# zhb94430/RayTracer-Utah

Hardware: AMD Instinct MI355X
Metric: Mrays/sec at 1920x1080 (the reference's primary + secondary + shadow rays of the frames rendered / wall time; batched throughput: config.frames_in_flight frames with their own cameras per launch sequence — one frame alone: config.single_frame) (higher is better)
Workload: dtype f32

## Files before the change

### include/rtu_render.h

```cpp
#ifndef RTU_RENDER_H_INCLUDED
#define RTU_RENDER_H_INCLUDED

#include "rtu_scene.h"

#ifdef __cplusplus
extern "C" {
#endif

#define RTU_OK               0
#define RTU_ERR_ARG         (-1)
#define RTU_ERR_HIP         (-2)
#define RTU_ERR_UNSUPPORTED (-3)
#define RTU_ERR_STOCHASTIC  (-4)
#define RTU_ERR_NO_SCENE    (-5)
#define RTU_ERR_NO_DEVICE   (-6)
#define RTU_ERR_CAPACITY    (-7)
#define RTU_ERR_CANCELLED   (-8)
#define RTU_ERR_SCENE_SHAPE (-9)
#define RTU_ERR_STALE       (-10)

#define RTU_BAND_ROWS 8

typedef struct RtuContext RtuContext;

// ... 142 lines not shown
int  rtu_light_list_info(const RtuContext* ctx, uint32_t index, uint32_t* out5);

typedef struct RtuLightListDump {
    int32_t  usable, node, light;
    uint32_t G, point, n_entries;
    float    X[3], Y[3], Z[3], L[3], u0, v0, su, sv;
    uint32_t* cell_off;
    uint32_t* entry_face;
    float*    entry_zmin;
} RtuLightListDump;
int  rtu_debug_light_list(const RtuSceneDesc* scene, uint32_t light_slot, uint32_t cover_slot, RtuLightListDump* out);
void rtu_debug_light_list_free(RtuLightListDump* dump);
int  rtu_debug_context_light_list(RtuContext* ctx, uint32_t index, RtuLightListDump* out);
int  rtu_debug_update_timing(RtuContext* ctx, int on, float* ms_out5);
int  rtu_debug_mesh_update_timing(RtuContext* ctx, int on, float* ms_out4);

#define RTU_MESH_BVH4          0
#define RTU_MESH_BVH8          1
#define RTU_MESH_FAST_TRI      2
#define RTU_MESH_REF_TRI       3
#define RTU_MESH_REF_BVH       4
#define RTU_MESH_REF_ELEMENTS  5
#define RTU_MESH_V             6
#define RTU_MESH_VN            7
#define RTU_MESH_HEADER        8
#define RTU_MESH_FAST_ELEMENTS 9
typedef struct RtuMeshHeaderDump {
    float    bmin[3], bmax[3], scale;
    uint32_t n_bvh_nodes, any_empty_box;
} RtuMeshHeaderDump;
int  rtu_debug_context_mesh(RtuContext* ctx, uint32_t mesh, int which, void* out, size_t capacity_bytes, size_t* bytes_out);
int  rtu_debug_host_mesh(const RtuMesh* uploaded, const RtuMesh* now, int which, void* out, size_t capacity_bytes, size_t* bytes_out);

int  rtu_frame_counts(RtuContext* ctx, uint32_t* frames_out, uint32_t* deferred_out);

int  rtu_get_stats(RtuContext* ctx, RtuStats* stats);

#define RTU_KERNEL_SLOTS 40
typedef struct RtuTouched {
    uint64_t rays;
    uint64_t node_tests, mesh_box_tests, inner4, inner8, inner_ref, tri_tests, winners, xform_levels;
    uint64_t record_bytes;
    uint64_t bound_tests;
    uint64_t inline_shadow_rays;
} RtuTouched;
int         rtu_get_touched(RtuContext* ctx, RtuTouched* per_slot, int n_slots);
int         rtu_get_touched_launches(RtuContext* ctx, uint32_t* per_slot, int n_slots);
unsigned long long rtu_touched_bytes(const RtuTouched* t, int textured);
const char* rtu_kernel_slot_name(int slot);

int  rtu_probe_kernel(RtuContext* ctx, int slot);
int  rtu_probe_read(RtuContext* ctx, float* total_ms_out, int* launches_out);

int  rtu_time_render(RtuContext* ctx, const RtuFrameDesc* frame, void* d_rgbz, void* hip_stream,
                     int iters, float* avg_ms_out);

int  rtu_selftest_division(RtuContext* ctx, unsigned long long n_pairs, unsigned long long seed,
                           unsigned long long* mismatches_out);

int  rtu_selftest_primitives(RtuContext* ctx, unsigned long long n_rays, unsigned long long seed,
                             unsigned long long* mismatches_out);

#define RTU_TEXOP_ATAN2F     0
#define RTU_TEXOP_ASINF      1
#define RTU_TEXOP_SPHERE_UV  2
#define RTU_TEXOP_ENV_UVW    3
// ... 25 lines not shown
```

### raytracer-utah_amd/__init__.py

```python
import ctypes
import os

_PKG = os.path.dirname(os.path.abspath(__file__))
_LIB = os.path.join(_PKG, "lib")

RTU_BIGFLOAT = 1.0e30
RTU_BAND_ROWS = 8

RTU_OK = 0
RTU_ERR_ARG = -1
RTU_ERR_HIP = -2
RTU_ERR_UNSUPPORTED = -3
RTU_ERR_STOCHASTIC = -4
RTU_ERR_NO_SCENE = -5
RTU_ERR_NO_DEVICE = -6
RTU_ERR_CAPACITY = -7
RTU_ERR_CANCELLED = -8
RTU_ERR_SCENE_SHAPE = -9
RTU_ERR_STALE = -10


class RtuError(RuntimeError):
    def __init__(self, code, msg=""):
        self.code = code
# ... 77 lines not shown


def _load(name):
    path = os.path.join(_LIB, name)
    if not os.path.exists(path):
        raise ImportError("%s is missing: build the HIP extension first (__graft_entry__.build() or "
                          "`make -C raytracer-utah_amd`); there is no CPU fallback" % path)
    return ctypes.CDLL(path, mode=ctypes.RTLD_GLOBAL)


hip = _load("librtu_hip.so")
host = _load("librtu_host.so")

_P = ctypes.c_void_p
_I = ctypes.c_int


def _sig(lib, name, restype, *argtypes):
    fn = getattr(lib, name)
    fn.restype = restype
    fn.argtypes = list(argtypes)
    return fn


HIP_SYMBOLS = ["rtu_device_count", "rtu_error_string", "rtu_create_context", "rtu_destroy_context", "rtu_last_error",
               "rtu_upload_scene", "rtu_validate_scene", "rtu_frame_setup", "rtu_shard_rows", "rtu_shard_max_rows", "rtu_shard_global_row",
               "rtu_render_frame_device", "rtu_render_frames_device", "rtu_pack_image_device", "rtu_minmax_z_device", "rtu_pack_output_device", "rtu_render_frame", "rtu_frame_status", "rtu_render_timeline", "rtu_frame_counts", "rtu_timeline_exits", "rtu_mesh_info", "rtu_light_list_info", "rtu_debug_light_list", "rtu_update_scene", "rtu_multi_update_scene", "rtu_scene_shape_diff", "rtu_debug_context_light_list", "rtu_debug_update_timing", "rtu_debug_light_list_free", "rtu_debug_walk_stack_limit", "rtu_debug_node_bounds", "rtu_debug_flags", "rtu_set_sequences_in_flight", "rtu_debug_tail_from", "rtu_get_stats", "rtu_get_touched", "rtu_get_touched_launches", "rtu_touched_bytes", "rtu_kernel_slot_name", "rtu_probe_kernel", "rtu_probe_read", "rtu_time_render", "rtu_selftest_division", "rtu_selftest_primitives", "rtu_context_stream", "rtu_context_device", "rtu_context_sync", "rtu_host_alloc_pinned", "rtu_host_free_pinned", "rtu_copy_to_host_async", "rtu_device_alloc",
               "rtu_device_free", "rtu_copy_to_host", "rtu_device_info", "rtu_set_cancel_flag", "rtu_create_context_multi", "rtu_destroy_context_multi",
               "rtu_multi_size", "rtu_multi_context", "rtu_multi_last_error", "rtu_multi_upload_scene", "rtu_multi_render_frame", "rtu_multi_gather_kind",
               "rtu_adaptive_defaults", "rtu_render_frame_adaptive", "rtu_render_frame_adaptive_device", "rtu_debug_sample_images", "rtu_debug_texcoords",
               "rtu_debug_device_allocations", "rtu_progressive_begin", "rtu_progressive_advance", "rtu_progressive_status",
               "rtu_progressive_snapshot_device", "rtu_progressive_snapshot", "rtu_progressive_free", "rtu_debug_device_bytes",
               "rtu_update_meshes", "rtu_multi_update_meshes", "rtu_debug_context_mesh", "rtu_debug_host_mesh", "rtu_debug_mesh_update_timing",
               "rtu_trace_rays_device", "rtu_occluded_rays_device", "rtu_trace_rays", "rtu_occluded_rays", "rtu_camera_rays"]
_sig(hip, "rtu_device_count", _I)
_sig(hip, "rtu_error_string", ctypes.c_char_p, _I)
_sig(hip, "rtu_create_context", _P, _I, ctypes.POINTER(_I))
_sig(hip, "rtu_destroy_context", None, _P)
_sig(hip, "rtu_last_error", ctypes.c_char_p, _P)
_sig(hip, "rtu_upload_scene", _I, _P, _P)
_sig(hip, "rtu_validate_scene", _I, _P, ctypes.c_char_p, ctypes.c_size_t)
_sig(hip, "rtu_frame_setup", _I, ctypes.POINTER(RtuCamera), _I, _I, ctypes.POINTER(RtuFrameDesc))
_sig(hip, "rtu_shard_rows", _I, ctypes.POINTER(RtuFrameDesc))
_sig(hip, "rtu_shard_max_rows", _I, _I, _I)
_sig(hip, "rtu_shard_global_row", _I, ctypes.POINTER(RtuFrameDesc), _I)
_sig(hip, "rtu_render_frame_device", _I, _P, ctypes.POINTER(RtuFrameDesc), _P, _P)
_sig(hip, "rtu_render_frames_device", _I, _P, ctypes.POINTER(RtuFrameDesc), _I, _P, _P)
_sig(hip, "rtu_pack_image_device", _I, _P, _P, ctypes.c_size_t, _P, _P, _P)
_sig(hip, "rtu_minmax_z_device", _I, _P, _P, ctypes.c_size_t, _I, _P, _P)
_sig(hip, "rtu_pack_output_device", _I, _P, _P, ctypes.c_size_t, _I, _P, _P, _P)
_sig(hip, "rtu_render_frame", _I, _P, ctypes.POINTER(RtuFrameDesc), _P, ctypes.POINTER(RtuStats))
_sig(hip, "rtu_frame_status", _I, _P)
_sig(hip, "rtu_get_touched", _I, _P, ctypes.POINTER(RtuTouched), _I)
_sig(hip, "rtu_touched_bytes", ctypes.c_uint64, ctypes.POINTER(RtuTouched), _I)
_sig(hip, "rtu_get_touched_launches", _I, _P, ctypes.POINTER(ctypes.c_uint32), _I)
_sig(hip, "rtu_kernel_slot_name", ctypes.c_char_p, _I)
_sig(hip, "rtu_probe_kernel", _I, _P, _I)
_sig(hip, "rtu_probe_read", _I, _P, ctypes.POINTER(ctypes.c_float), ctypes.POINTER(_I))
_sig(hip, "rtu_debug_walk_stack_limit", _I, _P, ctypes.c_uint32)
_sig(hip, "rtu_debug_node_bounds", _I, _P, _I)
_sig(hip, "rtu_debug_flags", _I, _P, ctypes.c_uint32)
_sig(hip, "rtu_set_sequences_in_flight", _I, _P, _I)
_sig(hip, "rtu_debug_tail_from", _I, _P, _I)
_sig(hip, "rtu_timeline_exits", _I, _P, _I, _I, ctypes.POINTER(ctypes.c_double))
_sig(hip, "rtu_mesh_info", _I, _P, ctypes.c_uint32, ctypes.POINTER(ctypes.c_uint32))
_sig(hip, "rtu_light_list_info", _I, _P, ctypes.c_uint32, ctypes.POINTER(ctypes.c_uint32))
_sig(hip, "rtu_frame_counts", _I, _P, ctypes.POINTER(ctypes.c_uint32), ctypes.POINTER(ctypes.c_uint32))
_sig(hip, "rtu_render_timeline", _I, _P, ctypes.POINTER(RtuFrameDesc), _P, _I, ctypes.POINTER(_I), ctypes.POINTER(ctypes.c_double),
     ctypes.POINTER(ctypes.c_double))
_sig(hip, "rtu_get_stats", _I, _P, ctypes.POINTER(RtuStats))
_sig(hip, "rtu_time_render", _I, _P, ctypes.POINTER(RtuFrameDesc), _P, _P, _I, ctypes.POINTER(ctypes.c_float))
_sig(hip, "rtu_selftest_primitives", _I, _P, ctypes.c_ulonglong, ctypes.c_ulonglong, ctypes.POINTER(ctypes.c_ulonglong))
_sig(hip, "rtu_selftest_division", _I, _P, ctypes.c_ulonglong, ctypes.c_ulonglong, ctypes.POINTER(ctypes.c_ulonglong))
_sig(hip, "rtu_device_alloc", _P, _P, ctypes.c_size_t)
_sig(hip, "rtu_device_free", None, _P, _P)
_sig(hip, "rtu_copy_to_host", _I, _P, _P, _P, ctypes.c_size_t)


class RtuAdaptiveDesc(ctypes.Structure):
    _fields_ = [("min_samples", ctypes.c_int32), ("increment", ctypes.c_int32), ("target_variance", ctypes.c_float), ("max_batch", ctypes.c_int32)]


RTU_MAX_BATCH = 16
_sig(hip, "rtu_adaptive_defaults", _I, ctypes.POINTER(RtuAdaptiveDesc))
_sig(hip, "rtu_render_frame_adaptive", _I, _P, ctypes.POINTER(RtuFrameDesc), ctypes.POINTER(RtuAdaptiveDesc), _P, _P, ctypes.POINTER(RtuStats))
_sig(hip, "rtu_render_frame_adaptive_device", _I, _P, ctypes.POINTER(RtuFrameDesc), ctypes.POINTER(RtuAdaptiveDesc), _P, _P, _P)
_sig(hip, "rtu_debug_sample_images", _I, _P, ctypes.POINTER(RtuFrameDesc), _I, _I, _P)
_sig(hip, "rtu_debug_texcoords", _I, _P, _I, _I, _P, ctypes.c_ulonglong, _P)
_sig(hip, "rtu_debug_device_allocations", ctypes.c_ulonglong)
_sig(hip, "rtu_debug_device_bytes", ctypes.c_ulonglong)
_sig(hip, "rtu_progressive_begin", _P, _P, ctypes.POINTER(RtuFrameDesc), ctypes.POINTER(RtuAdaptiveDesc), ctypes.POINTER(_I))
_sig(hip, "rtu_progressive_advance", _I, _P, _I, _P)
_sig(hip, "rtu_progressive_status", _I, _P, ctypes.POINTER(ctypes.c_int32), ctypes.POINTER(ctypes.c_uint32))
_sig(hip, "rtu_progressive_snapshot_device", _I, _P, _P, _P, _P)
_sig(hip, "rtu_progressive_snapshot", _I, _P, _P, _P)
_sig(hip, "rtu_progressive_free", None, _P)
TEXOP_ATAN2F, TEXOP_ASINF, TEXOP_SPHERE_UV, TEXOP_ENV_UVW, TEXOP_TILE_CLAMP, TEXOP_TEXTURE, TEXOP_MAP = range(7)
TEXOP_IN = (2, 1, 3, 3, 3, 3, 3)
TEXOP_OUT = (1, 1, 3, 3, 3, 3, 3)

# ... 618 lines not shown
        if rc < 0:
            self._check(rc)
        order = {name: i for i, name in enumerate(self.TIMELINE_SLOTS)}
        rows = [(self.TIMELINE_SLOTS[slot[i]], t0[i], t1[i]) for i in range(rc)]
        return sorted(rows, key=lambda r: (r[0].startswith("k_combine"), -order[r[0]] if r[0].startswith("k_combine") else order[r[0]]))

    def timeline_exits(self, kernel):
        import numpy as np
        buf = (ctypes.c_double * 8192)()
        rc = hip.rtu_timeline_exits(self._h, self.TIMELINE_SLOTS.index(kernel), 8192, buf)
        if rc < 0:
            self._check(rc)
        return np.array(buf[:rc])

    def mesh_info(self, mesh=0):
        o = (ctypes.c_uint32 * 5)()
        self._check(hip.rtu_mesh_info(self._h, mesh, o))
        return dict(zip(("faces", "sah_depth", "stack4", "nodes4", "nodes8"), list(o)))

    def light_lists(self):
        out, i = [], 0
        while True:
            o = (ctypes.c_uint32 * 5)()
            if hip.rtu_light_list_info(self._h, i, o) != 0:
                return out
            out.append(dict(zip(("light", "cover", "G", "entries", "longest"), list(o))))
            i += 1

    def frame_counts(self):
        fr, de = (ctypes.c_uint32 * 6)(), (ctypes.c_uint32 * 7)()
        self._check(hip.rtu_frame_counts(self._h, fr, de))
        return list(fr), list(de)

    def time_render(self, frame, d_ptr, stream, iters):
        ms = ctypes.c_float(0)
        self._check(hip.rtu_time_render(self._h, ctypes.byref(frame), d_ptr, stream, iters, ctypes.byref(ms)))
        return ms.value

    def touched(self, textured=False):
        arr = (RtuTouched * KERNEL_SLOTS)()
        n = hip.rtu_get_touched(self._h, arr, KERNEL_SLOTS)
        if n < 0:
            self._check(n)
        nl = (ctypes.c_uint32 * KERNEL_SLOTS)()
        hip.rtu_get_touched_launches(self._h, nl, KERNEL_SLOTS)
        out = {}
        for k in range(n):
            d = arr[k].as_dict()
            if any(d.values()):
                d["bytes"] = int(hip.rtu_touched_bytes(ctypes.byref(arr[k]), 1 if textured else 0))
                d["launches"] = int(nl[k])
                out[hip.rtu_kernel_slot_name(k).decode()] = d
        return out

    def probe_kernel(self, slot_name):
        slot = -1
        if slot_name is not None:
            names = [hip.rtu_kernel_slot_name(k).decode() for k in range(KERNEL_SLOTS)]
            slot = names.index(slot_name)
        self._check(hip.rtu_probe_kernel(self._h, slot))

    def probe_read(self):
        ms, n = ctypes.c_float(0), _I(0)
        self._check(hip.rtu_probe_read(self._h, ctypes.byref(ms), ctypes.byref(n)))
        return ms.value, n.value

# ... 110 lines not shown
```

### raytracer-utah_amd/csrc/render_impl.h

```cpp
#ifndef RTU_RENDER_IMPL_H_INCLUDED
#define RTU_RENDER_IMPL_H_INCLUDED
#include "rtu_intersect.h"

namespace {

#define TEXD ((TEX & 1) != 0)
#define SMPD ((TEX & 2) != 0)
#define BATD ((TEX & 4) != 0)
#define GID ((TEX & 8) != 0)
#define CNTD ((TEX & 16) != 0)
#ifndef RTU_OCC_PRIMARY
#define RTU_OCC_PRIMARY __attribute__((amdgpu_waves_per_eu(4, 4)))
#endif
#ifndef RTU_OCC_PRIMARY_S
#define RTU_OCC_PRIMARY_S __attribute__((amdgpu_waves_per_eu(5, 5)))
#endif
#ifndef RTU_OCC_TRACE
#define RTU_OCC_TRACE __attribute__((amdgpu_waves_per_eu(5, 5)))
#endif
#ifndef RTU_OCC_WALK
#define RTU_OCC_WALK __attribute__((amdgpu_waves_per_eu(3, 3)))
#endif
#ifndef RTU_OCC_CONSUME
#define RTU_OCC_CONSUME
// ... 378 lines not shown
            if (GID) {
                a.gi_h[pix] = make_float4(h.p.x, h.p.y, h.p.z, h.z);
                a.gi_h[pix + a.gi_total] = make_float4(h.N.x, h.N.y, h.N.z, __uint_as_float((want ? 1u : 0u) | (h.front ? 2u : 0u) | ((uint32_t)(mid + 1) << 2)));
                a.gi_h[pix + 2u * (size_t)a.gi_total] = make_float4(ray.dir.x, ray.dir.y, ray.dir.z, __uint_as_float(smp.key));
                if (TEXD) a.gi_h[pix + 3u * (size_t)a.gi_total] = make_float4(h.uvw.x, h.uvw.y, h.uvw.z, 0.0f);
                RTU_BYTES(TEXD ? 64u : 48u);
                want = false;
            }
        }
    }
    if (GID) return;
    uint32_t info = 0;
    if (want) info = make_info<TEX>(a, mid, a.frame.max_bounce, h.front, ray.dir, h.p, h.N, h.uvw, smp);
    if (!STATS && INLINE_SHADE && !(a.dbg & 2048u) && __any(want && !(info & (RTU_FI_MAIN | RTU_FI_C)))) {
        const bool tryI = want && !(info & (RTU_FI_MAIN | RTU_FI_C));
        uint32_t lit = ~0u;
        bool ok = false;
        if (tryI) ok = shadows_inline<TEX>(a, info, h.p, lit, cnt);
        if (tryI && ok) {
            f3 direct = mk3(0, 0, 0);
            if (info & RTU_FI_SH) {
                const f3 cam_pos = BATD ? ld3(a.cam[sidx].pos) : ld3(a.frame.cam_pos);
                direct = direct_light<false, TEX>(a, info, h.p, h.N, h.uvw, cam_pos, direct, [&](uint32_t j) { return ((lit >> j) & 1u) ? 1.0f : 0.0f; });
            }
            a.out[pix] = make_float4(direct.x, direct.y, direct.z, h.z);
            RTU_BYTES(16u);
            want = false;
        }
    }
    if (!(a.dbg & 8u)) append_root<TEX>(a, want, shard, info, h.p, h.N, pix, ray.dir, h.z, h.uvw, cnt, !DEFER && !STATS);
    if (CNTD && !DEFER && !COOP && (a.dbg & 131072u) && valid) a.out[pix].x = (float)walk_units;
}

template <int STACK, bool STATS, int TEX>
__device__ __forceinline__ void primary_stage1(const KernelArgs& a, uint32_t n_tiles) {
    const Stamp stamp(a, RTU_TL_PRIMARY);
    __shared__ uint32_t s_stack_all[STATS ? 4 * STACK * 64 : 4];
    uint32_t* stk = s_stack_all + (STATS ? (threadIdx.x >> 6) * (STACK * 64) + (threadIdx.x & 63u) : 0);
    const uint32_t lane = threadIdx.x & 63u;
    Counters cnt = {};
    const uint32_t wave = (uint32_t)__builtin_amdgcn_readfirstlane((int)(threadIdx.x >> 6));
    for (uint32_t btile = blockIdx.x * 4u + wave; btile < n_tiles; btile += gridDim.x * 4u) {
        uint32_t sidx = (SMPD || BATD) ? btile / a.tiles_per_image : 0u;
        uint32_t tile = btile - sidx * a.tiles_per_image;
        bool lane_on = true;
        if constexpr (SMPD) {
            if (a.act_list != nullptr) {
                sidx = btile / a.act_n;
                const RTU_CONST uint32_t* ent = as_const(reinterpret_cast<const uint32_t*>(a.act_list)) + 4u * (size_t)(btile - sidx * a.act_n);
                tile = ent[0];
                lane_on = (((unsigned long long)ent[3] << 32 | ent[2]) >> lane) & 1ull;
            }
        }
        const uint32_t band_local = tile / a.tiles_x;
        const uint32_t tx = tile - band_local * a.tiles_x;
        const int x = (int)(tx * 8 + (lane & 7));
        const int ly = (int)(band_local * RTU_BAND_ROWS + (lane >> 3));
        const int y = (int)((band_local * a.frame.shard_count + a.frame.shard_rank) * RTU_BAND_ROWS + (lane >> 3));
        const bool valid = x < a.frame.width && y < a.frame.height && lane_on;
        const uint32_t pix = ((SMPD || BATD) ? sidx * a.batch_pixels : 0u) + (uint32_t)ly * (uint32_t)a.frame.width + (uint32_t)x;
        if (!STATS && !SMPD && !GID && a.occ != nullptr) {
            const uint32_t w = as_const(a.occ)[(size_t)sidx * a.occ_words + (tile >> 5)];
            if (!((w >> (tile & 31u)) & 1u)) {
                if (valid) {
                    const f3 bg = background_sample<TEXD>(a.scene, x, y);
                    a.out[pix] = make_float4(bg.x, bg.y, bg.z, RTU_BIGFLOAT);
                    RTU_BYTES(16u);
                    if (CNTD) cnt.t_rays++;
                }
                if (CNTD && lane == 0) cnt.t_bytes += 4u;
                continue;
            }
        }
        const uint32_t shard = btile % RTU_SHARDS;
        bool deferred;
        primary_pixel<STACK, STATS, !STATS, false, TEX, RTU_INLINE_PRIMARY>(a, valid, x, y, sidx, pix, shard, stk, cnt, deferred);
        if (!STATS && !(a.dbg & 8u)) defer_push(a, 0, shard, deferred, pix);
        if (deferred) RTU_BYTES(4u);
    }
    flush_counters<STATS>(a, cnt);
    flush_touched<TEX>(a, cnt, RTU_TL_PRIMARY);
}
template <int STACK, bool STATS, int TEX>
__global__ void __launch_bounds__(256) RTU_OCC_PRIMARY k_primary(KernelArgs a, uint32_t n_tiles) { primary_stage1<STACK, STATS, TEX>(a, n_tiles); }
template <int STACK, int TEX>
__global__ void __launch_bounds__(256) RTU_OCC_PRIMARY_S k_primary_sampled(KernelArgs a, uint32_t n_tiles) { primary_stage1<STACK, false, TEX>(a, n_tiles); }
template <int STACK, int TEX>
__global__ void __launch_bounds__(256) k_primary_counting(KernelArgs a, uint32_t n_tiles) { primary_stage1<STACK, true, TEX>(a, n_tiles); }

__device__ __forceinline__ void stage_nodes(const KernelArgs& a, float4* lds_nodes) {
    const RTU_CONST DevMesh* meshes = as_const(a.scene.meshes);
    for (uint32_t m = 0; m < a.n_meshes; m++) {
        const float4* src = meshes[m].bvh8;
        const uint32_t n = meshes[m].lds_nodes * 16u, off = meshes[m].lds_off;
// ... 1001 lines not shown
    const uint32_t nm = a.cover ? entries * a.scene.n_cover : 0u, np = a.cover ? entries * a.scene.n_pcover : 0u;
    if (blockIdx.y < nm) mesh_cover_body(a, entries, blockIdx.y);
    else if (blockIdx.y < nm + np) plane_cover_body(a, entries, blockIdx.y - nm);
    else if (blockIdx.x == 0u) node_rects_body(a, entries);
}

__global__ void __launch_bounds__(64) k_tile_occ(KernelArgs a, uint32_t entries) {
    const uint32_t e = blockIdx.y;
    if (e >= entries) return;
    const DevScene& s = a.scene;
    const uint32_t tiles = a.tiles_per_image;
    const uint32_t tile = blockIdx.x * 64u + threadIdx.x;
    bool occ = false;
    if (tile < tiles) {
        const uint32_t band_local = tile / a.tiles_x, tx = tile - band_local * a.tiles_x;
        const int x0 = (int)(tx * 8u), y0 = (int)((band_local * (uint32_t)a.frame.shard_count + (uint32_t)a.frame.shard_rank) * RTU_BAND_ROWS);
        const int x1 = x0 + 8 < a.frame.width ? x0 + 8 : a.frame.width, y1 = y0 + 8 < a.frame.height ? y0 + 8 : a.frame.height;
        const uint32_t gtile = (uint32_t)(y0 >> 3) * a.tiles_xf + tx;
        for (uint32_t k = 0; k < s.n_nodes && k < 64u; k++) {
            if (!((s.obj_mask >> k) & 1ull)) continue;
            const int4 r = a.node_rects[(size_t)e * s.n_nodes + k];
            if (!(x0 < r.z && x1 > r.x && y0 < r.w && y1 > r.y)) continue;
            bool masked_out = false;
            if (a.cover)
                for (uint32_t c = 0; c < s.n_cover + s.n_pcover; c++)
                    if ((uint32_t)(c < s.n_cover ? s.cover_node[c] : s.pcover_node[c - s.n_cover]) == k) {
                        const uint32_t* m = a.cover + ((size_t)e * (s.n_cover + s.n_pcover) + c) * (1u + a.cover_words);
                        if (m[0] == 0u && !((m[1u + (gtile >> 5)] >> (gtile & 31u)) & 1u)) masked_out = true;
                    }
            if (!masked_out) occ = true;
        }
    }
    const unsigned long long bits = __ballot(occ);
    if (threadIdx.x == 0) {
        uint32_t* o = const_cast<uint32_t*>(a.occ) + (size_t)e * a.occ_words + 2u * blockIdx.x;
        o[0] = (uint32_t)bits;
        o[1] = (uint32_t)(bits >> 32);
        if (bits) atomicAdd(&a.fcnt->occ_tiles[((blockIdx.x + 7u * blockIdx.y) % RTU_SHARDS) * RTU_CSTRIDE], (uint32_t)__popcll(bits));
    }
}

#define RTU_LAUNCH_ON(strm_, kslot_, kernel, grid, blk, ...)                                  \
    do {                                                                                     \
        const bool probed_ = probe && probe->slot == (kslot_);                               \
        if (a.host_launches) a.host_launches[(kslot_)]++;                                    \
        if (probed_) (void)hipEventRecord((hipEvent_t)probe->ev0, (strm_));                  \
        hipLaunchKernelGGL(kernel, grid, blk, 0, (strm_), __VA_ARGS__);                      \
        if (probed_) { (void)hipEventRecord((hipEvent_t)probe->ev1, (strm_)); if (probe->recorded) *probe->recorded = 1; } \
    } while (0)
#define RTU_LAUNCH(kslot_, kernel, grid, blk, ...) RTU_LAUNCH_ON(stream, kslot_, kernel, grid, blk, __VA_ARGS__)

template <int STACK, int TEX>
int launch_all(const KernelArgs& a, uint32_t n_tiles, bool stats, hipStream_t stream, int mode = RTU_LAUNCH_ALL, const LaunchProbe* probe = nullptr) {
    const int levels = a.frame.max_bounce + 1;
    const dim3 block(64);
    const dim3 gridT(32768), gridN(32768), gridS(8192), gridF0(16384), gridF(4096), gridC(1024), gridCoop(512);
    const uint32_t thr = (uint32_t)(a.frame.coop_threshold > 0 ? a.frame.coop_threshold : 70000);
    auto grid_lane = [&](int ph, dim3 full) {
        const uint32_t n1 = ph < 8 ? a.list_n[ph] : 0u;
        if (n1 == 0u || n1 - 1u > thr) return full;
        uint32_t g = ((n1 - 1u + 63u) / 64u) * 2u;
        g = g < 2048u ? 2048u : g;
        return g < full.x ? dim3(g) : full;
    };
    auto grid_coop = [&](int ph) {
        const uint32_t n1 = ph < 8 ? a.list_n[ph] : 0u;
        return (n1 != 0u && n1 - 1u > 2u * (uint64_t)thr) ? dim3(16) : gridCoop;
    };
    auto grid_coop2 = [&](int ph) {
        const uint32_t n1 = ph < 8 ? a.list_n[ph] : 0u;
        return (n1 != 0u && n1 - 1u > 2u * (uint64_t)thr) ? dim3(32) : dim3(2u * gridCoop.x);
// ... 80 lines not shown
```

### raytracer-utah_amd/csrc/rtu_capi.hip

```cpp
#include "rtu_devbuf.h"
#include "rtu_device.h"
#include "rtu_lightlist.h"
#include "rtu_meshrec.h"
#include "rtu_query.h"

#include <algorithm>
#include <array>
#include <cmath>
#include <cstdarg>
#include <cstdio>
#include <cstdlib>
#include <cstring>
#include <map>
#include <memory>
#include <string>
#include <vector>

struct RtuProgressive;

struct RtuContext {
    int         device = 0;
    hipStream_t stream = nullptr;
    hipStream_t aux_stream = nullptr;
    hipEvent_t  aux_ev0 = nullptr, aux_ev1 = nullptr;
// ... 57 lines not shown
    DevBuf<float4>   gi_res;
    bool      want_gi = false;
    int      tail_hint = 0, last_tail_from = RTU_MAX_LEVELS;
    std::map<uint64_t, int> tail_hints;
    std::map<uint64_t, std::array<uint32_t, 8>> list_hints;
    uint64_t last_tail_key = 0;
    bool     last_stats = false;
    uint32_t n_meshes = 0;
    uint32_t nsl = 0;
    int32_t  shadow_light[RTU_MAX_SHADOW_LIGHTS] = {};
    float    nol_light[RTU_FI_NOL_LIGHTS][4] = {};
    DevBuf<float4> fb;
    DevBuf<unsigned long long> counters;
    uint32_t slot_launches[RTU_TL_KERNELS] = {};
    static const int kProbePairs = 64;
    int probe_slot = -1, probe_used = 0;
    hipEvent_t probe_ev[2 * kProbePairs] = {};
    struct MeshInfo { uint32_t faces, sah_depth, stack4, nodes4, nodes8; };
    std::vector<MeshInfo> mesh_info;
    struct LightListInfo { uint32_t light, cover, G, entries, longest; };
    std::vector<LightListInfo> light_list_info;
    static const int kCamSlots = 16;
    DevBuf<BatchCam> d_cams;
    PinnedBuf<BatchCam> h_cams;
    hipEvent_t cam_ev[kCamSlots] = {};
    int cam_slot = 0;
    uint32_t dbg = 0;
    const volatile int* cancel = nullptr;
    uint64_t scene_gen = 0;
    std::vector<RtuProgressive*> sessions;
    DevBuf<uint32_t> cover;
    uint32_t  cover_faces = 0;
    DevBuf<uint32_t> occ;
    int4* node_rects = nullptr;
    DevBuf<float4>  q_rays, q_hits;
    DevBuf<uint8_t> q_occ;
    DevBuf<unsigned long long> tl;
    bool stamp_next = false;
};

namespace {

const size_t kCounterBytes = (size_t)RTU_TL_KERNELS * RTU_TOUCH_STRIDE * sizeof(unsigned long long);

int fail(RtuContext* ctx, int code, const char* fmt, ...) {
    char buf[512];
    va_list ap;
    va_start(ap, fmt);
    vsnprintf(buf, sizeof buf, fmt, ap);
    va_end(ap);
    if (ctx) ctx->error = buf;
    return code;
}

#define RTU_HIP(ctx, call)                                                                        \
    do {                                                                                          \
        hipError_t e_ = (call);                                                                   \
        if (e_ != hipSuccess) return fail(ctx, RTU_ERR_HIP, "%s: %s", #call, hipGetErrorString(e_)); \
    } while (0)

void free_scene(RtuContext* ctx) {
    ctx->scene_allocs.clear();
    ctx->place.clear();
    ctx->has_scene = false;
}

// ... 893 lines not shown
    memcpy(a.lv, ctx->lv, sizeof a.lv);
    a.fcnt = ctx->fcnt.get();
    a.tl = ctx->stamp_next ? ctx->tl.get() : nullptr;
    a.defer_list = ctx->defer_list;
    a.defer_cap_s = ctx->defer_cap_s;
    a.defer_list0 = ctx->defer_list0;
    a.defer_cap0_s = ctx->defer_cap0_s;
    a.fcnt0 = ctx->fcnt.get();
    a.dbg = ctx->dbg;
    a.scene.dbg = ctx->dbg;
    a.counters = stats ? ctx->counters.get() : nullptr;
    a.host_launches = stats == 2 ? ctx->slot_launches : nullptr;
    a.node_rects = (stats != 1 && frame->samples == 0 && ctx->dscene.node_bounds) ? ctx->node_rects : nullptr;
    if (a.node_rects && (ctx->dscene.n_cover + ctx->dscene.n_pcover) && !gi && ((size_t)((frame->width + 7) / 8) * (size_t)((frame->height + 7) / 8) + 31u) / 32u <= 12288u) {
        a.tiles_xf = (uint32_t)((frame->width + 7) / 8);
        a.cover_words = (a.tiles_xf * (uint32_t)((frame->height + 7) / 8) + 31u) / 32u;
        a.cover_faces = ctx->cover_faces;
        const size_t need = (size_t)batch * (ctx->dscene.n_cover + ctx->dscene.n_pcover) * (1u + a.cover_words);
        if (need > ctx->cover.size()) {
            RTU_HIP(ctx, hipStreamSynchronize(stream));
            RTU_HIP(ctx, ctx->cover.grow(need));
        }
        RTU_HIP(ctx, hipMemsetAsync(ctx->cover.get(), 0, need * sizeof(uint32_t), stream));
        a.cover = ctx->cover.get();
    }
    if (a.node_rects && !gi && ctx->dscene.n_nodes <= 64u && stats != 1 && !(ctx->dbg & 256u)) {
        a.occ_words = ((tiles_x * bands + 63u) / 64u) * 2u;
        const size_t need = (size_t)batch * a.occ_words;
        if (need > ctx->occ.size()) {
            RTU_HIP(ctx, hipStreamSynchronize(stream));
            RTU_HIP(ctx, ctx->occ.grow(need));
        }
        a.occ = a.occ_words ? ctx->occ.get() : nullptr;
    }
    a.tiles_x = tiles_x;
    a.tiles_per_image = tiles_x * bands;
    a.nsl = ctx->nsl;
    a.n_meshes = ctx->n_meshes;
    const uint32_t act_tiles = act_n ? act_n * (uint32_t)batch : n_tiles;
    const uint64_t tail_key = adaptive ? ((uint64_t)(32 - __builtin_clz(act_tiles | 1u)) << 8) | (uint64_t)(16 | 2 | (gi ? 8 : 0))
                                       : ((uint64_t)n_tiles << 8) | (uint64_t)((frame->samples ? 2 : 0) | (frames_batch ? 4 : 0) | (gi ? 8 : 0));
    int hint = RTU_MAX_LEVELS;
    bool forced = false;
    if (ctx->tail_hint != 0) { hint = ctx->tail_hint; ctx->tail_hint = 0; forced = true; }
    else if (ctx->tail_hints.count(tail_key)) hint = ctx->tail_hints[tail_key];
    a.tail_from = stats == 1 ? RTU_MAX_LEVELS : hint;
    ctx->last_tail_key = tail_key;
    if (stats == 0 && !gi && !(ctx->dbg & 512u) && ctx->list_hints.count(tail_key)) memcpy(a.list_n, ctx->list_hints[tail_key].data(), sizeof a.list_n);
    if (forced) a.dbg |= 128u;
    if (frame->samples >= 1) {
        const float pixelIncrement = (float)(1.0 / frame->samples);
        a.sampling = 1;
        a.sample_index = (uint32_t)sample_index;
        a.batch = (uint32_t)batch;
        a.batch_pixels = pixels;
        a.tiles_per_image = tiles_x * bands;
        for (int b = 0; b < batch; b++) {
            const int index = sample_index + b;
            const float currentOffset = (float)index * pixelIncrement;
            a.pix_off_x[b] = currentOffset + halton(index, 4);
            a.pix_off_y[b] = currentOffset + halton(index, 5);
        }
    }
    if (frames_batch) {
        a.frame_batch = 1;
        a.batch = (uint32_t)batch;
        a.batch_pixels = pixels;
// ... 19 lines not shown
    }
    if (gi) {
        a.gi_h = ctx->gi_h.get();
        a.gi_res = ctx->gi_res.get();
        a.gi_depth = (uint32_t)gi_depth;
        a.gi_total = pixels * (uint32_t)batch;
    }
    const uint32_t launch_tiles = act_list ? act_n * (uint32_t)batch : n_tiles;
    a.act_list = act_list;
    a.act_n = act_n;
    ctx->last_side = false;
    const uint32_t thr0 = (uint32_t)(frame->coop_threshold > 0 ? frame->coop_threshold : 70000);
    if (stats != 1 && !gi && frame->samples == 0 && ctx->n_meshes > 0 && ctx->mesh_hits_childless && !ctx->stamp_next && !(ctx->dbg & (8192u | 2048u | 64u)) &&
        ctx->dscene.node_bounds && ctx->dscene.lmask &&
        !ctx->side_off.count(tail_key) && ctx->list_hints.count(tail_key) && ctx->list_hints[tail_key][0] - 1u > thr0 &&
        ctx->side_frames.count(tail_key) && ctx->side_frames[tail_key] <= 256u) {
        if (!ctx->aux_stream) {
            int prio_least = 0, prio_greatest = 0;
            RTU_HIP(ctx, hipDeviceGetStreamPriorityRange(&prio_least, &prio_greatest));
            RTU_HIP(ctx, hipStreamCreateWithPriority(&ctx->aux_stream, hipStreamNonBlocking, prio_least));
            RTU_HIP(ctx, hipEventCreateWithFlags(&ctx->aux_ev0, hipEventDisableTiming));
            RTU_HIP(ctx, hipEventCreateWithFlags(&ctx->aux_ev1, hipEventDisableTiming));
        }
        a.side = 1;
        a.fcnt0 = ctx->fcnt_side.get();
        memcpy(a.lv_side, ctx->lv_side, sizeof a.lv_side);
        a.aux_stream = ctx->aux_stream;
        a.aux_ev0 = ctx->aux_ev0;
        a.aux_ev1 = ctx->aux_ev1;
        RTU_HIP(ctx, hipMemsetAsync(ctx->fcnt_side.get(), 0, offsetof(FrameCounters, overflow), stream));
        ctx->last_side = true;
    }
    a.pgrid = 32768u;
    if (a.occ && !(ctx->dbg & 512u) && ctx->occ_hints.count(tail_key) && (uint64_t)ctx->occ_hints[tail_key] * 3u < (uint64_t)n_tiles)
        a.pgrid = ctx->sequences_in_flight >= 2 ? 1024u : 4096u;
    ctx->last_tail_from = a.tail_from;
    ctx->last_stats = stats == 1;
    memcpy(a.shadow_light, ctx->shadow_light, sizeof a.shadow_light);
    memcpy(a.nol_light, ctx->nol_light, sizeof a.nol_light);
    int probe_recorded = 0;
    LaunchProbe probe{-1, nullptr, nullptr, &probe_recorded};
    const bool probing = ctx->probe_slot >= 0 && ctx->probe_used < RtuContext::kProbePairs;
    if (probing) {
        probe.slot = ctx->probe_slot;
        probe.ev0 = ctx->probe_ev[2 * ctx->probe_used];
        probe.ev1 = ctx->probe_ev[2 * ctx->probe_used + 1];
    }
    if (gi_mode == RTU_LAUNCH_SHADE && gi_depth == 0) {
        hipError_t e0 = (hipError_t)rtu_launch_frame(a, launch_tiles, ctx->bvh_stack_needed, stats, stream, gi_mode, probing ? &probe : nullptr);
        if (probing && probe_recorded) ctx->probe_used++;
        if (e0 != hipSuccess) return fail(ctx, RTU_ERR_HIP, "kernel launch: %s", hipGetErrorString(e0));
        e0 = (hipError_t)rtu_launch_gi_final(a, stream);
        if (e0 != hipSuccess) return fail(ctx, RTU_ERR_HIP, "kernel launch: %s", hipGetErrorString(e0));
        return RTU_OK;
    }
    hipError_t e = (hipError_t)rtu_launch_frame(a, launch_tiles, ctx->bvh_stack_needed, stats, stream, gi_mode, probing ? &probe : nullptr);
    if (probing && probe_recorded) ctx->probe_used++;
    if (e != hipSuccess) return fail(ctx, RTU_ERR_HIP, "kernel launch: %s", hipGetErrorString(e));
    return RTU_OK;
}

uint64_t stage2_total(const FrameCounters& h) {
    uint64_t n = 0;
    for (int s = 0; s < RTU_SHARDS; s++) n += h.stage2_frames[s * RTU_CSTRIDE];
    return n;
}

// ... 1709 lines not shown

int rtu_light_list_info(const RtuContext* ctx, uint32_t index, uint32_t* out5) {
    if (!ctx || !out5) return RTU_ERR_ARG;
    if (index >= ctx->light_list_info.size()) return RTU_ERR_ARG;
    const RtuContext::LightListInfo& i = ctx->light_list_info[index];
    out5[0] = i.light; out5[1] = i.cover; out5[2] = i.G; out5[3] = i.entries; out5[4] = i.longest;
    return RTU_OK;
}

int rtu_frame_counts(RtuContext* ctx, uint32_t* frames_out, uint32_t* deferred_out) {
    if (!ctx || !frames_out || !deferred_out) return RTU_ERR_ARG;
    RTU_HIP(ctx, hipSetDevice(ctx->device));
    RTU_HIP(ctx, hipDeviceSynchronize());
    std::unique_ptr<FrameCounters> hp(new FrameCounters);
    FrameCounters& h = *hp;
    RTU_HIP(ctx, hipMemcpy(&h, ctx->fcnt.get(), sizeof h, hipMemcpyDeviceToHost));
    for (int L = 0; L < RTU_MAX_LEVELS; L++) {
        frames_out[L] = 0;
        for (int s = 0; s < RTU_SHARDS; s++) frames_out[L] += h.n_frames[L][(s) * RTU_CSTRIDE];
    }
    for (int p = 0; p <= RTU_MAX_LEVELS; p++) {
        deferred_out[p] = 0;
        for (int s = 0; s < RTU_SHARDS; s++) deferred_out[p] += h.n_defer[p][(s) * RTU_CSTRIDE];
    }
    if (ctx->last_side) {
        RTU_HIP(ctx, hipMemcpy(&h, ctx->fcnt_side.get(), sizeof h, hipMemcpyDeviceToHost));
        for (int L = 0; L < RTU_MAX_LEVELS; L++)
            for (int s = 0; s < RTU_SHARDS; s++) frames_out[L] += h.n_frames[L][(s) * RTU_CSTRIDE];
        for (int s = 0; s < RTU_SHARDS; s++) deferred_out[0] += h.n_defer[0][(s) * RTU_CSTRIDE];
    }
    return RTU_OK;
}

int rtu_selftest_division(RtuContext* ctx, unsigned long long n_pairs, unsigned long long seed, unsigned long long* mismatches_out) {
    if (!ctx || !mismatches_out) return RTU_ERR_ARG;
    RTU_HIP(ctx, hipSetDevice(ctx->device));
    RTU_HIP(ctx, hipMemsetAsync(ctx->counters.get(), 0, sizeof(unsigned long long), ctx->stream));
    hipError_t e = (hipError_t)rtu_launch_selftest_fdiv(n_pairs, seed, ctx->counters.get(), ctx->stream);
    if (e != hipSuccess) return fail(ctx, RTU_ERR_HIP, "selftest launch: %s", hipGetErrorString(e));
    RTU_HIP(ctx, hipStreamSynchronize(ctx->stream));
    RTU_HIP(ctx, hipMemcpy(mismatches_out, ctx->counters.get(), sizeof(unsigned long long), hipMemcpyDeviceToHost));
    return RTU_OK;
}

int rtu_selftest_primitives(RtuContext* ctx, unsigned long long n_rays, unsigned long long seed, unsigned long long* mismatches_out) {
    if (!ctx || !mismatches_out) return RTU_ERR_ARG;
    RTU_HIP(ctx, hipSetDevice(ctx->device));
    RTU_HIP(ctx, hipMemsetAsync(ctx->counters.get(), 0, sizeof(unsigned long long), ctx->stream));
    hipError_t e = (hipError_t)rtu_launch_selftest_prims(n_rays, seed, ctx->counters.get(), ctx->stream);
    if (e != hipSuccess) return fail(ctx, RTU_ERR_HIP, "selftest launch: %s", hipGetErrorString(e));
    RTU_HIP(ctx, hipStreamSynchronize(ctx->stream));
    RTU_HIP(ctx, hipMemcpy(mismatches_out, ctx->counters.get(), sizeof(unsigned long long), hipMemcpyDeviceToHost));
    return RTU_OK;
}

int rtu_debug_texcoords(RtuContext* ctx, int op, int index, const float* h_in, unsigned long long n, float* h_out) {
    if (!ctx) return RTU_ERR_ARG;
    if (op < RTU_TEXOP_ATAN2F || op > RTU_TEXOP_MAP) return fail(ctx, RTU_ERR_ARG, "unknown texcoords op %d", op);
    if (n && (!h_in || !h_out)) return fail(ctx, RTU_ERR_ARG, "h_in / h_out is NULL");
    const DevTexture* tex = nullptr;
    RtuTexMap map;
    const DevScene& s = ctx->dscene;
    if (op == RTU_TEXOP_TEXTURE || op == RTU_TEXOP_MAP) {
        if (!ctx->has_scene) return fail(ctx, RTU_ERR_NO_SCENE, "no scene uploaded");
        if (ctx->n_textures == 0) return fail(ctx, RTU_ERR_ARG, "the uploaded scene has no textures");
        if (op == RTU_TEXOP_TEXTURE) {
// ... 185 lines not shown
```

### raytracer-utah_amd/csrc/rtu_device.h

```cpp
#ifndef RTU_DEVICE_H_INCLUDED
#define RTU_DEVICE_H_INCLUDED

#include "rtu_render.h"
#include "rtu_vec.h"

__device__ __forceinline__ int cvtt_i32(float v) { return (v > -2147483904.0f && v < 2147483648.0f) ? (int)v : (int)0x80000000; }

#define RTU_CONST __attribute__((address_space(4)))
template <class T> __device__ __forceinline__ const RTU_CONST T* as_const(const T* p) {
#pragma clang diagnostic push
#pragma clang diagnostic ignored "-Wold-style-cast"
    return (const RTU_CONST T*)(p);
#pragma clang diagnostic pop
}

#define RTU_GLOBAL __attribute__((address_space(1)))
typedef float rtu_v4f __attribute__((ext_vector_type(4)));
struct GBase {
    const RTU_GLOBAL char* p;
};
template <class T> __device__ __forceinline__ GBase global_base(const T* ptr) {
    const unsigned long long b = (unsigned long long)ptr;
    const unsigned lo = (unsigned)__builtin_amdgcn_readfirstlane((int)(unsigned)b), hi = (unsigned)__builtin_amdgcn_readfirstlane((int)(unsigned)(b >> 32));
    GBase g;
// ... 189 lines not shown
    uint32_t*    defer_list0;
    uint32_t     defer_cap0_s, side;
    uint32_t     pgrid, pad_pg;
    void*        aux_stream;
    void*        aux_ev0;
    void*        aux_ev1;
    uint32_t     dbg;
    uint32_t*    cover;
    uint32_t     cover_words, tiles_xf;
    uint32_t     cover_faces, pad_cf;
    int4*        node_rects;
    const uint32_t* occ;
    uint32_t     occ_words, pad_occ;
    unsigned long long* counters;
    uint32_t     tiles_x;
    uint32_t     nsl;
    int32_t      shadow_light[RTU_MAX_SHADOW_LIGHTS];
    float        nol_light[RTU_FI_NOL_LIGHTS][4];
    uint32_t     n_meshes;
    int32_t      tail_from;
    uint32_t     list_n[8];
    uint32_t*    host_launches;
    uint32_t     sampling;
    uint32_t     sample_index;
    uint32_t     batch, batch_pixels, tiles_per_image;
    float        pix_off_x[RTU_MAX_BATCH], pix_off_y[RTU_MAX_BATCH];
    float4*      gi_h;
    float4*      gi_res;
    uint32_t     gi_depth, gi_total;
    uint32_t     frame_batch;
    const BatchCam* cam;
    const uint4* act_list;
    uint32_t     act_n, pad_act;
};

#define RTU_LAUNCH_ALL   0
#define RTU_LAUNCH_CHAIN 1
#define RTU_LAUNCH_SHADE 2
#define RTU_GI_BOUNCES   4
struct LaunchProbe {
    int   slot;
    void* ev0;
    void* ev1;
    int*  recorded;
};
int rtu_launch_frame(const KernelArgs& args, uint32_t n_tiles, uint32_t bvh_stack_needed, int stats, hipStream_t stream, int mode = RTU_LAUNCH_ALL,
                     const LaunchProbe* probe = nullptr);
int rtu_launch_gi_final(const KernelArgs& args, hipStream_t stream);

int rtu_launch_accumulate(const float4* samples, uint32_t batch, float4* acc, uint32_t* hits, uint32_t pixels, bool first, hipStream_t stream);
int rtu_launch_resolve(const float4* acc, const uint32_t* hits, float4* out, uint32_t pixels, uint32_t samples, hipStream_t stream);
struct AdaptiveStep {
    const float4* samples;
    float4* acc;
    float4* sq;
    uint32_t* hits;
    uint8_t* counts;
    const uint4* list_in;
    uint4* list_out;
    uint32_t* n_out;
    const uint32_t* skip_if;
    const uint32_t* skip_if_side;
    uint32_t n_in, batch, first, pixels;
    int32_t width, height, shard_rank, shard_count;
    uint32_t tiles_x, min_samples, increment, max_samples;
    float target;
// ... 19 lines not shown
```

Before: 60620.

## Compact occupied tiles into sharded list for primary stage iteration

The occupancy kernel now also writes the indices of occupied tiles into a per-shard compacted list, using atomic bases and ballot prefix counts. The primary stage walks this list, found through a wave-level prefix scan of the shard counts, instead of scanning every tile and testing occupancy bits. Empty tiles are filled with background by a separate bitmask-word walk that is interleaved with the list walk. The primary grid size becomes smaller when the list is active, and a debug API is added to read the list back. The cost is extra global writes and list memory, plus more complex load balancing between the two walks.

```diff
diff --git a/include/rtu_render.h b/include/rtu_render.h
--- a/include/rtu_render.h
+++ b/include/rtu_render.h
@@ -198,6 +198,8 @@
 int  rtu_debug_context_mesh(RtuContext* ctx, uint32_t mesh, int which, void* out, size_t capacity_bytes, size_t* bytes_out);
 int  rtu_debug_host_mesh(const RtuMesh* uploaded, const RtuMesh* now, int which, void* out, size_t capacity_bytes, size_t* bytes_out);
 
+int  rtu_debug_tile_list(RtuContext* ctx, uint32_t* entries_out, uint32_t capacity, uint32_t* n_out, uint32_t* occ_tiles_out);
+
 int  rtu_frame_counts(RtuContext* ctx, uint32_t* frames_out, uint32_t* deferred_out);
 
 int  rtu_get_stats(RtuContext* ctx, RtuStats* stats);
diff --git a/raytracer-utah_amd/__init__.py b/raytracer-utah_amd/__init__.py
--- a/raytracer-utah_amd/__init__.py
+++ b/raytracer-utah_amd/__init__.py
@@ -133,7 +133,7 @@
                "rtu_debug_device_allocations", "rtu_progressive_begin", "rtu_progressive_advance", "rtu_progressive_status",
                "rtu_progressive_snapshot_device", "rtu_progressive_snapshot", "rtu_progressive_free", "rtu_debug_device_bytes",
                "rtu_update_meshes", "rtu_multi_update_meshes", "rtu_debug_context_mesh", "rtu_debug_host_mesh", "rtu_debug_mesh_update_timing",
-               "rtu_trace_rays_device", "rtu_occluded_rays_device", "rtu_trace_rays", "rtu_occluded_rays", "rtu_camera_rays"]
+               "rtu_trace_rays_device", "rtu_occluded_rays_device", "rtu_trace_rays", "rtu_occluded_rays", "rtu_camera_rays", "rtu_debug_tile_list"]
 _sig(hip, "rtu_device_count", _I)
 _sig(hip, "rtu_error_string", ctypes.c_char_p, _I)
 _sig(hip, "rtu_create_context", _P, _I, ctypes.POINTER(_I))
@@ -167,6 +167,7 @@
 _sig(hip, "rtu_mesh_info", _I, _P, ctypes.c_uint32, ctypes.POINTER(ctypes.c_uint32))
 _sig(hip, "rtu_light_list_info", _I, _P, ctypes.c_uint32, ctypes.POINTER(ctypes.c_uint32))
 _sig(hip, "rtu_frame_counts", _I, _P, ctypes.POINTER(ctypes.c_uint32), ctypes.POINTER(ctypes.c_uint32))
+_sig(hip, "rtu_debug_tile_list", _I, _P, ctypes.POINTER(ctypes.c_uint32), ctypes.c_uint32, ctypes.POINTER(ctypes.c_uint32), ctypes.POINTER(ctypes.c_uint32))
 _sig(hip, "rtu_render_timeline", _I, _P, ctypes.POINTER(RtuFrameDesc), _P, _I, ctypes.POINTER(_I), ctypes.POINTER(ctypes.c_double),
      ctypes.POINTER(ctypes.c_double))
 _sig(hip, "rtu_get_stats", _I, _P, ctypes.POINTER(RtuStats))
@@ -851,6 +852,15 @@
         self._check(hip.rtu_frame_counts(self._h, fr, de))
         return list(fr), list(de)
 
+    def tile_list(self):
+        import numpy as np
+        n, counted = ctypes.c_uint32(0), ctypes.c_uint32(0)
+        hip.rtu_debug_tile_list(self._h, None, 0, ctypes.byref(n), ctypes.byref(counted))
+        out = np.empty(n.value, np.uint32)
+        if n.value:
+            self._check(hip.rtu_debug_tile_list(self._h, out.ctypes.data_as(ctypes.POINTER(ctypes.c_uint32)), n.value, ctypes.byref(n), ctypes.byref(counted)))
+        return out[:n.value], counted.value
+
     def time_render(self, frame, d_ptr, stream, iters):
         ms = ctypes.c_float(0)
         self._check(hip.rtu_time_render(self._h, ctypes.byref(frame), d_ptr, stream, iters, ctypes.byref(ms)))
diff --git a/raytracer-utah_amd/csrc/render_impl.h b/raytracer-utah_amd/csrc/render_impl.h
--- a/raytracer-utah_amd/csrc/render_impl.h
+++ b/raytracer-utah_amd/csrc/render_impl.h
@@ -434,6 +434,35 @@
     if (CNTD && !DEFER && !COOP && (a.dbg & 131072u) && valid) a.out[pix].x = (float)walk_units;
 }
 
+template <int TEX>
+__device__ __forceinline__ void background_word(const KernelArgs& a, uint32_t wi, uint32_t lane, Counters& cnt) {
+    const uint32_t sidx = BATD ? wi / a.occ_words : 0u;
+    const uint32_t tile0 = (wi - sidx * a.occ_words) * 32u;
+    if (tile0 >= a.tiles_per_image) return;
+    uint32_t clear = ~as_const(a.occ)[wi];
+    if (CNTD && lane == 0) cnt.t_bytes += 4u;
+    if (a.tiles_per_image - tile0 < 32u) clear &= (1u << (a.tiles_per_image - tile0)) - 1u;
+    if (clear == 0u) return;
+    uint32_t band_local = tile0 / a.tiles_x, tx = tile0 - band_local * a.tiles_x, at = 0;
+    while (clear != 0u) {
+        const uint32_t bit = (uint32_t)__builtin_ctz(clear);
+        clear &= clear - 1u;
+        tx += bit - at;
+        at = bit;
+        while (tx >= a.tiles_x) { tx -= a.tiles_x; band_local++; }
+        const int x = (int)(tx * 8 + (lane & 7));
+        const int ly = (int)(band_local * RTU_BAND_ROWS + (lane >> 3));
+        const int y = (int)((band_local * a.frame.shard_count + a.frame.shard_rank) * RTU_BAND_ROWS + (lane >> 3));
+        const uint32_t pix = (BATD ? sidx * a.batch_pixels : 0u) + (uint32_t)ly * (uint32_t)a.frame.width + (uint32_t)x;
+        if (x < a.frame.width && y < a.frame.height) {
+            const f3 bg = background_sample<TEXD>(a.scene, x, y);
+            a.out[pix] = make_float4(bg.x, bg.y, bg.z, RTU_BIGFLOAT);
+            RTU_BYTES(16u);
+            if (CNTD) cnt.t_rays++;
+        }
+    }
+}
+
 template <int STACK, bool STATS, int TEX>
 __device__ __forceinline__ void primary_stage1(const KernelArgs& a, uint32_t n_tiles) {
     const Stamp stamp(a, RTU_TL_PRIMARY);
@@ -442,7 +471,47 @@
     const uint32_t lane = threadIdx.x & 63u;
     Counters cnt = {};
     const uint32_t wave = (uint32_t)__builtin_amdgcn_readfirstlane((int)(threadIdx.x >> 6));
-    for (uint32_t btile = blockIdx.x * 4u + wave; btile < n_tiles; btile += gridDim.x * 4u) {
+    constexpr bool LISTABLE = !STATS && !SMPD && !GID;
+    static_assert(RTU_SHARDS == 64, "one segment per lane");
+    bool listed = false;
+    uint32_t n_list = 0, n_words = 0, wi = 0, per = 1;
+    uint32_t* seg_end = nullptr;
+    if constexpr (LISTABLE) {
+        __shared__ uint32_t s_seg_end[4 * RTU_SHARDS];
+        seg_end = s_seg_end + wave * RTU_SHARDS + lane;
+        if (a.occ != nullptr && a.occ_list != nullptr && !(a.dbg & 1024u)) {
+            listed = true;
+            const uint32_t first = blockIdx.x * 4u + wave, step = gridDim.x * 4u;
+            wi = first;
+            uint32_t end = a.fcnt->occ_tiles[lane * RTU_CSTRIDE];
+            end = end < a.occ_list_cap_s ? end : a.occ_list_cap_s;
+#pragma unroll
+            for (int off = 1; off < 64; off <<= 1) {
+                const uint32_t below = (uint32_t)__shfl_up((int)end, off);
+                if (lane >= (uint32_t)off) end += below;
+            }
+            *seg_end = end;
+            n_list = (uint32_t)__builtin_amdgcn_readlane((int)end, 63);
+            n_words = (BATD ? a.batch : 1u) * a.occ_words;
+            const uint32_t my_entries = n_list > first ? (n_list - first + step - 1u) / step : 0u;
+            const uint32_t my_words = n_words > first ? (n_words - first + step - 1u) / step : 0u;
+            per = my_entries ? (my_words + my_entries - 1u) / my_entries : 1u;
+        }
+    }
+    for (uint32_t it = blockIdx.x * 4u + wave; (LISTABLE && listed) || it < n_tiles; it += gridDim.x * 4u) {
+        uint32_t btile = it;
+        if (LISTABLE && listed) {
+            for (uint32_t k = 0; k < per && wi < n_words; k++, wi += gridDim.x * 4u) background_word<TEX>(a, wi, lane, cnt);
+            if (it >= n_list) {
+                if (wi >= n_words) break;
+                continue;
+            }
+            const uint32_t end = *seg_end;
+            const uint32_t seg = (uint32_t)__ffsll((long long)__ballot(end > it)) - 1u;
+            const uint32_t seg_begin = seg ? (uint32_t)__builtin_amdgcn_readlane((int)end, (int)(seg - 1u)) : 0u;
+            btile = (uint32_t)__builtin_amdgcn_readfirstlane((int)as_const(a.occ_list)[(size_t)seg * a.occ_list_cap_s + (it - seg_begin)]);
+            if (CNTD && lane == 0) cnt.t_bytes += 4u;
+        }
         uint32_t sidx = (SMPD || BATD) ? btile / a.tiles_per_image : 0u;
         uint32_t tile = btile - sidx * a.tiles_per_image;
         bool lane_on = true;
@@ -461,7 +530,7 @@
         const int y = (int)((band_local * a.frame.shard_count + a.frame.shard_rank) * RTU_BAND_ROWS + (lane >> 3));
         const bool valid = x < a.frame.width && y < a.frame.height && lane_on;
         const uint32_t pix = ((SMPD || BATD) ? sidx * a.batch_pixels : 0u) + (uint32_t)ly * (uint32_t)a.frame.width + (uint32_t)x;
-        if (!STATS && !SMPD && !GID && a.occ != nullptr) {
+        if (!STATS && !SMPD && !GID && a.occ != nullptr && !listed) {
             const uint32_t w = as_const(a.occ)[(size_t)sidx * a.occ_words + (tile >> 5)];
             if (!((w >> (tile & 31u)) & 1u)) {
                 if (valid) {
@@ -1529,11 +1598,17 @@
         }
     }
     const unsigned long long bits = __ballot(occ);
+    const uint32_t shard = (blockIdx.y * gridDim.x + blockIdx.x) % RTU_SHARDS;
+    uint32_t base = 0;
     if (threadIdx.x == 0) {
         uint32_t* o = const_cast<uint32_t*>(a.occ) + (size_t)e * a.occ_words + 2u * blockIdx.x;
         o[0] = (uint32_t)bits;
         o[1] = (uint32_t)(bits >> 32);
-        if (bits) atomicAdd(&a.fcnt->occ_tiles[((blockIdx.x + 7u * blockIdx.y) % RTU_SHARDS) * RTU_CSTRIDE], (uint32_t)__popcll(bits));
+        if (bits) base = atomicAdd(&a.fcnt->occ_tiles[shard * RTU_CSTRIDE], (uint32_t)__popcll(bits));
+    }
+    if (a.occ_list != nullptr && bits) {
+        const uint32_t idx = (uint32_t)__shfl((int)base, 0) + (uint32_t)__popcll(bits & ((1ull << threadIdx.x) - 1ull));
+        if (occ && idx < a.occ_list_cap_s) a.occ_list[(size_t)shard * a.occ_list_cap_s + idx] = e * tiles + tile;
     }
 }
 
diff --git a/raytracer-utah_amd/csrc/rtu_capi.hip b/raytracer-utah_amd/csrc/rtu_capi.hip
--- a/raytracer-utah_amd/csrc/rtu_capi.hip
+++ b/raytracer-utah_amd/csrc/rtu_capi.hip
@@ -113,6 +113,8 @@
     DevBuf<uint32_t> cover;
     uint32_t  cover_faces = 0;
     DevBuf<uint32_t> occ;
+    DevBuf<uint32_t> occ_list;
+    uint32_t  last_list_cap_s = 0;
     int4* node_rects = nullptr;
     DevBuf<float4>  q_rays, q_hits;
     DevBuf<uint8_t> q_occ;
@@ -1072,7 +1074,18 @@
             RTU_HIP(ctx, ctx->occ.grow(need));
         }
         a.occ = a.occ_words ? ctx->occ.get() : nullptr;
-    }
+        if (a.occ && !(ctx->dbg & 1024u)) {
+            const uint32_t wavefronts = (a.occ_words / 2u) * (uint32_t)batch;
+            a.occ_list_cap_s = ((wavefronts + RTU_SHARDS - 1u) / RTU_SHARDS) * 64u;
+            const size_t need_list = (size_t)RTU_SHARDS * a.occ_list_cap_s;
+            if (need_list > ctx->occ_list.size()) {
+                RTU_HIP(ctx, hipStreamSynchronize(stream));
+                RTU_HIP(ctx, ctx->occ_list.grow(need_list));
+            }
+            a.occ_list = ctx->occ_list.get();
+        }
+    }
+    ctx->last_list_cap_s = a.occ_list ? a.occ_list_cap_s : 0u;
     a.tiles_x = tiles_x;
     a.tiles_per_image = tiles_x * bands;
     a.nsl = ctx->nsl;
@@ -1158,7 +1171,10 @@
         ctx->last_side = true;
     }
     a.pgrid = 32768u;
-    if (a.occ && !(ctx->dbg & 512u) && ctx->occ_hints.count(tail_key) && (uint64_t)ctx->occ_hints[tail_key] * 3u < (uint64_t)n_tiles)
+    static const uint32_t kListGridEnv = [] { const char* e = getenv("RTU_PRIMARY_LIST_GRID"); return e ? (uint32_t)strtoul(e, nullptr, 10) : 0u; }();
+    if (a.occ_list)
+        a.pgrid = kListGridEnv ? kListGridEnv : (ctx->sequences_in_flight >= 2 ? 1024u : 2048u);
+    else if (a.occ && !(ctx->dbg & 512u) && ctx->occ_hints.count(tail_key) && (uint64_t)ctx->occ_hints[tail_key] * 3u < (uint64_t)n_tiles)
         a.pgrid = ctx->sequences_in_flight >= 2 ? 1024u : 4096u;
     ctx->last_tail_from = a.tail_from;
     ctx->last_stats = stats == 1;
@@ -2934,6 +2950,30 @@
     return RTU_OK;
 }
 
+int rtu_debug_tile_list(RtuContext* ctx, uint32_t* entries_out, uint32_t capacity, uint32_t* n_out, uint32_t* occ_tiles_out) {
+    if (!ctx || !n_out || (capacity && !entries_out)) return RTU_ERR_ARG;
+    RTU_HIP(ctx, hipSetDevice(ctx->device));
+    RTU_HIP(ctx, hipDeviceSynchronize());
+    std::unique_ptr<FrameCounters> hp(new FrameCounters);
+    RTU_HIP(ctx, hipMemcpy(hp.get(), ctx->fcnt.get(), sizeof(FrameCounters), hipMemcpyDeviceToHost));
+    const uint32_t cap_s = ctx->last_list_cap_s;
+    uint64_t counted = 0, n = 0;
+    for (int s = 0; s < RTU_SHARDS; s++) {
+        const uint32_t c = hp->occ_tiles[s * RTU_CSTRIDE];
+        counted += c;
+        n += c < cap_s ? c : cap_s;
+    }
+    *n_out = (uint32_t)n;
+    if (occ_tiles_out) *occ_tiles_out = (uint32_t)counted;
+    if (n > capacity) return capacity ? fail(ctx, RTU_ERR_ARG, "rtu_debug_tile_list: %llu entries, room for %u", (unsigned long long)n, capacity) : RTU_ERR_ARG;
+    for (int s = 0; s < RTU_SHARDS; s++) {
+        const uint32_t c = hp->occ_tiles[s * RTU_CSTRIDE] < cap_s ? hp->occ_tiles[s * RTU_CSTRIDE] : cap_s;
+        if (c) RTU_HIP(ctx, hipMemcpy(entries_out, ctx->occ_list.get() + (size_t)s * cap_s, c * sizeof(uint32_t), hipMemcpyDeviceToHost));
+        entries_out += c;
+    }
+    return RTU_OK;
+}
+
 int rtu_selftest_division(RtuContext* ctx, unsigned long long n_pairs, unsigned long long seed, unsigned long long* mismatches_out) {
     if (!ctx || !mismatches_out) return RTU_ERR_ARG;
     RTU_HIP(ctx, hipSetDevice(ctx->device));
diff --git a/raytracer-utah_amd/csrc/rtu_device.h b/raytracer-utah_amd/csrc/rtu_device.h
--- a/raytracer-utah_amd/csrc/rtu_device.h
+++ b/raytracer-utah_amd/csrc/rtu_device.h
@@ -245,6 +245,8 @@
     const BatchCam* cam;
     const uint4* act_list;
     uint32_t     act_n, pad_act;
+    uint32_t*    occ_list;
+    uint32_t     occ_list_cap_s, pad_ol;
 };
 
 #define RTU_LAUNCH_ALL   0
```

After: 59440. 0.981x the previous value.
